# Fabstir/fabstir-vectordb

Measured on AMD Instinct MI355X. Metric: k-NN queries/sec at recall@10>=0.95, 1Mx384 f32, higher is better.
Workload: dtype f32

## Files before the change

### fabstir-vectordb_amd/csrc/fvdb_hip.cpp

```cpp
#include "fvdb_internal.h"

#include <unistd.h>

#include <algorithm>
#include <atomic>
#include <cmath>
#include <condition_variable>
#include <mutex>
#include <cstdio>
#include <cstdlib>
#include <cstring>
#include <map>
#include <new>
#include <string>
#include <vector>

#include "common.h"
#include "pool.h"
#include "kernels_misc.h"
#include "kernels_scan.h"
#include "kernels_wide.h"
#include "kernels_range.h"
#include "kernels_rank.h"
#include "kernels_curve.h"
#include "kernels_coarse.h"
#include "kernels_mfma.h"
#include "kernels_mfma_wg.h"
#include "kernels_util.h"
#include "kernels_maint.h"
#include "kernels_rows.h"
#include "kernels_mmr.h"
#include "kernels_group.h"

using namespace fvdb;


enum FbWord : uint32_t {
  FB_COARSE = 0,
  FB_SCAN = 1,
  FB_REASONS = 2,
  FB_OVERFLOW = 2,
  FB_REFINED = 6,
  FB_WORDS = 8,
};
constexpr size_t kFbBytes = FB_WORDS * 4;
constexpr size_t kFbAllBytes = 2 * kFbBytes;
constexpr uint32_t kFbReasonWords = 5;

enum StageEvent {
  EV_COARSE_BEGIN = 0,
  EV_COARSE_SCANNED,
  EV_COARSE_DONE,
  EV_SCAN_BEGIN,
  EV_SCAN_DONE,
  EV_FINE_DONE,
  EV_FILTER_BEGIN,
  EV_FILTER_DONE,
  EV_COUNT
};

enum ScalWord : uint32_t {
  SC_COARSE_ITEMS = 0,
  SC_COARSE_HEAD = 1,
  SC_FINE_ITEMS = 2,
  SC_FINE_HEAD = 3,
  SC_STATS = 4,
};
constexpr size_t kScalarsBytes = 64;

struct IvfScratch {
  std::mutex enq;
  bool pend_filter = false;
  bool pending_profile = false, pend_coarse = false, pend_fine = false, collecting = false;
  DBuf s_qnorm, s_A;
  DBuf s_qh, s_qn2, s_thr, s_tA, s_pa, s_surv, s_scnt, s_fail, s_mslots;
  DBuf s_sdist, s_probes2;
  DBuf s_q, s_cpart, s_probes, s_cnt, s_fill, s_eoff, s_ioff, s_entries;
  DBuf s_part, s_scalars, s_ceoff, s_cioff;
  DBuf s_wbase, s_arena;
  DBuf s_wgbase;
  DBuf s_gwords, s_group;
  DBuf s_rbase, s_rarena;
  DBuf s_qual;
  DBuf s_clive, s_cprobes, s_ckeys, s_cval;
  DBuf s_in, s_slots, s_ids, s_clusters, s_out_ids, s_out_dist, s_out_cnt, s_cdist;
  DBuf s_fslots, s_frows;
  DevEvent fetch_done;
  DevEvent sev[EV_COUNT];
  uint32_t* scalar(ScalWord w) const { return s_scalars.as<uint32_t>() + w; }
};

struct fvdb_ivf : IvfScratch {
  static constexpr uint32_t kSlots = 16;
  IvfScratch spare[kSlots - 1];
  static constexpr uint32_t kLeases = 8;
  IvfScratch lease_set[kLeases];
  fvdb_ctx* lease_ctx[kLeases] = {};
  uint32_t lease_busy = 0;
  std::mutex mu;
  std::condition_variable lease_cv;
  std::atomic<IvfScratch*> last_set{nullptr};
  std::atomic<fvdb_ctx*> last_ctx{nullptr};
  fvdb_ctx* ctx = nullptr;
  uint32_t d = 0, dpad = 0, d4 = 0, nlist = 0;
  bool trained = false;
  bool f16 = false;

  std::vector<float> h_centroids;
  DBuf d_centroids_rm;
  DBuf d_cent_pad;
  DBuf d_cnorm, d_cnmax;
  DBuf s_fallbacks;
  uint32_t* fb_word(FbWord w, bool masked = false) const { return s_fallbacks.as<uint32_t>() + (masked ? FB_WORDS : 0) + w; }
  int coarse_mode = 0;
  int scan_mode = 0;
  HBuf h_fb;
  uint64_t mfma_q = 0;
  uint64_t fb_seen = 0, q_seen = 0;
  uint32_t exact_batches_left = 0;
  uint32_t backoff_len = 0;
  uint64_t overflow_seen = 0, overflow_q = 0;
  uint32_t refine_batches_left = 0;
  DBuf d_mfma_stamps;
  int mfma_stamps_launch = 0;
  DBuf d_xmax;
  Pool cpool;
  DBuf c_off, c_blocks, c_glob;

  Pool pool;
// ... 8 lines not shown
  bool glob_set = false;

  DBuf m_seq, m_dest, m_ids;
  fvdb_ivf* m_src = nullptr;
  uint64_t m_rows = 0;
  bool m_assigned = false;
  bool m_store_job = false;
  fvdb_maintenance_info_t m_info{};

  fvdb_search_stats last_stats{};
  float stage_ms[8] = {0, 0, 0, 0, 0, 0, 0, 0};
  uint64_t stage_calls = 0;
};

namespace {
struct Env {
  fvdb_ctx* ctx;
  IvfScratch* S;
  const uint64_t* live = nullptr;
};
inline IvfScratch& slot_scratch(fvdb_ivf* ivf, uint32_t slot) { return slot == 0 ? *ivf : ivf->spare[slot - 1]; }
inline const uint64_t* live_words(const fvdb_ivf* ivf, const Env& E) { return E.live ? E.live : ivf->pool.valid(); }
inline PoolView list_pool(const fvdb_ivf* ivf, const Env& E) {
  PoolView v = ivf->pool.view();
  v.valid = live_words(ivf, E);
  return v;
}
}


namespace {

struct IvfKnobs {
  static int num(const char* name, int unset) { return getenv(name) ? atoi(getenv(name)) : unset; }
  static bool has(const char* name) { return getenv(name) != nullptr; }
  static int tiles(int m) { return m >= 4 ? 4 : (m >= 2 ? 2 : 1); }
  bool coarse_exact = has("FVDB_COARSE_EXACT");
  bool scan_exact = has("FVDB_SCAN_EXACT");
  uint32_t scan_wgs_per_cu = (uint32_t)num("FVDB_SCAN_WGS_PER_CU", 8);
  int segb = num("FVDB_SEGB", 0);
  bool no_shared_thr = has("FVDB_NO_SHARED_THR");
  int mfma_m = tiles(num("FVDB_MFMA_M", 2));
  int mfma_segb = num("FVDB_MFMA_SEGB", 0);
  uint32_t mfma_wgs_per_cu = (uint32_t)std::max(1, num("FVDB_MFMA_WGS_PER_CU", 2));
  bool mfma_groups_in_item = num("FVDB_MFMA_GROUPS_IN_ITEM", 0) != 0;
  bool mfma_wg = num("FVDB_MFMA_WG", 1) != 0;
  int mfma_wg_m = num("FVDB_MFMA_WG_M", 4) >= 4 ? 4 : 2;
  uint32_t mfma_wg_segb = (uint32_t)std::max(4, num("FVDB_MFMA_WG_SEGB", 16));
  uint32_t mfma_wg_per_cu = (uint32_t)std::max(1, num("FVDB_MFMA_WG_PER_CU", 2));
  int mfma_wg_tail_pct = num("FVDB_MFMA_WG_TAIL_PCT", 25);
  int mfma_wg_segb_tail = num("FVDB_MFMA_WG_SEGB_TAIL", 4);
  uint32_t mfma_cap_a = (uint32_t)std::max(1, num("FVDB_MFMA_CAP_A", 4));
  bool mfma_threshold_pass = has("FVDB_MFMA_THRESHOLD_PASS");
  uint32_t mfma_segb_a = (uint32_t)std::max(1, num("FVDB_MFMA_SEGB_A", 1));
  bool mfma_no_refine = has("FVDB_MFMA_NO_REFINE");
#ifdef FVDB_MFMA_STAMPS_BUILD
  int mfma_stamps = num("FVDB_MFMA_STAMPS", 0);
#endif
};
const IvfKnobs& ivf_knobs() {
  static const IvfKnobs knobs{};
  return knobs;
}

struct ScanLaunch {
  PoolView pool;
  const uint32_t* list_off;
  const uint32_t* list_blocks;
  uint32_t nlist;
  const uint32_t* entry_off;
  const uint32_t* item_off;
  const uint2* entries;
  const uint32_t* n_items;
  uint32_t* head;
  const float* queries;
  uint32_t dpad, segb, k, nprobe, maxsegs;
  uint2* part;
  uint32_t max_items = 0;
  bool f16 = false;
};

inline int kr_for(uint32_t k) { return k <= 64 ? 1 : (k <= 128 ? 2 : 4); }
inline uint32_t q_for(uint32_t k) { return k <= 64 ? 16u : (k <= 128 ? 8u : 4u); }

template <int Q, int KR, int ROLE, int ST>
void launch_scan_t(fvdb_ctx* ctx, const ScanLaunch& s) {
  uint32_t grid = (uint32_t)ctx->num_cus * ivf_knobs().scan_wgs_per_cu;
  if (s.max_items) grid = std::min(grid, std::max<uint32_t>(1u, (s.max_items + 3) / 4));
  hipLaunchKernelGGL((scan_topk_kernel<Q, KR, ROLE, ST>), dim3(grid), dim3(256), 0, ctx->stream, s.pool.data, s.pool.valid,
                     s.pool.d4, s.list_off, s.list_blocks, s.nlist, s.entry_off, s.item_off, (const u32x2*)s.entries,
                     s.n_items, s.head, s.queries, s.dpad, s.segb, s.k, s.nprobe, s.maxsegs, (u32x2*)s.part);
}

template <int ROLE, int ST>
void launch_scan_rs(fvdb_ctx* ctx, const ScanLaunch& s) {
  switch (kr_for(s.k)) {
    case 1: launch_scan_t<16, 1, ROLE, ST>(ctx, s); break;
    case 2: launch_scan_t<8, 2, ROLE, ST>(ctx, s); break;
    default: launch_scan_t<4, 4, ROLE, ST>(ctx, s); break;
  }
}
template <int ROLE>
void launch_scan_r(fvdb_ctx* ctx, const ScanLaunch& s) {
  if (s.f16) launch_scan_rs<ROLE, 1>(ctx, s); else launch_scan_rs<ROLE, 0>(ctx, s);
}
enum { ROLE_COARSE = 0, ROLE_LIST = 1, ROLE_ALL = 2 };
// ... 288 lines not shown
constexpr uint32_t kMfmaSlack = 6;
constexpr uint32_t kMfmaCmax = 4096;

bool mfma_shape_ok(const fvdb_ivf* ivf, uint32_t B, uint32_t k, uint32_t np) {
  return ivf->dpad % 16 == 0 && k + kMfmaSlack <= 32 && np <= 256 && B >= 32 && B <= 16384;
}
inline bool half_rows(const fvdb_ivf* ivf) { return ivf->f16 || ivf->pool.half() != nullptr; }
inline int x_rounded(const fvdb_ivf* ivf) { return ivf->f16 ? 0 : (ivf->pool.half() ? 1 : 2); }

struct MfmaPlan {
  bool wg;
  int M;
  uint32_t Q, ka, cmax;
  uint32_t segb, segbA;
  uint32_t lsplit, segb_tail;
  uint32_t fsegb, fmaxsegs;
  uint64_t fpart;
  uint32_t grid, wg_grid, wg_lds;
  bool half_rows;
  int x_rounded;
};

int mfma_plan(fvdb_ivf* ivf, fvdb_ctx* ctx, const IvfKnobs& kn, uint32_t B, uint32_t k, uint32_t np, MfmaPlan* out) {
  MfmaPlan P{};
  P.half_rows = half_rows(ivf);
  P.x_rounded = x_rounded(ivf);
  int wgM = kn.mfma_wg_m;
  if (mfma_wg_lds_bytes(ivf->dpad, 16u * wgM) > 64u * 1024u) wgM = 2;
  P.wg = kn.mfma_wg && kn.mfma_m == 2 && P.half_rows && ivf->dpad % 128 == 0 &&
         mfma_wg_lds_bytes(ivf->dpad, 16u * wgM) <= 64u * 1024u;
  P.M = P.wg ? wgM : kn.mfma_m;
  P.Q = 16u * P.M;
  P.ka = k + kMfmaSlack;
  P.cmax = kMfmaCmax;
  P.segbA = kn.mfma_segb_a;
  P.segb = P.wg ? kn.mfma_wg_segb : (kn.mfma_segb > 0 ? (uint32_t)kn.mfma_segb : pick_segb(ivf, B, np));
  P.lsplit = 0xFFFFFFFFu;
  P.segb_tail = P.segb;
  if (P.wg && kn.mfma_wg_tail_pct > 0 && kn.mfma_wg_segb_tail > 0 && (uint32_t)kn.mfma_wg_segb_tail < P.segb) {
    P.lsplit = (uint32_t)((uint64_t)ivf->nlist * (uint32_t)(100 - std::min(kn.mfma_wg_tail_pct, 100)) / 100);
    P.segb_tail = (uint32_t)kn.mfma_wg_segb_tail;
  }
  P.fsegb = pick_segb(ivf, B, np);
  P.fmaxsegs = std::max<uint32_t>(1, cdiv(ivf->max_list_blocks, P.fsegb));
  P.fpart = (uint64_t)B * np * P.fmaxsegs * k;
  if (P.fpart >= (1ull << 32)) FAIL(ctx, FVDB_E_UNSUPPORTED, "batch too large for one launch (sub-batch it)");
  P.grid = (uint32_t)ctx->num_cus * kn.mfma_wgs_per_cu;
  P.wg_grid = (uint32_t)ctx->num_cus * kn.mfma_wg_per_cu;
  P.wg_lds = mfma_wg_lds_bytes(ivf->dpad, P.Q);
  *out = P;
  return FVDB_OK;
}

int mfma_scratch(fvdb_ivf* ivf, const Env& E, const MfmaPlan& P, uint32_t B, uint32_t np) {
  fvdb_ctx* ctx = E.ctx;
  IvfScratch& S = *E.S;
  HIPCHK(ctx, S.s_qh.ensure((size_t)(B + 1) * ivf->dpad * 2));
  HIPCHK(ctx, S.s_qn2.ensure((size_t)B * 4));
  HIPCHK(ctx, S.s_thr.ensure((size_t)B * 4));
  HIPCHK(ctx, S.s_tA.ensure((size_t)B * 4));
  HIPCHK(ctx, S.s_pa.ensure((size_t)B * 4));
  HIPCHK(ctx, S.s_mslots.ensure((size_t)B * 64 * 4));
  HIPCHK(ctx, S.s_surv.ensure((size_t)B * P.cmax * 8));
  HIPCHK(ctx, S.s_sdist.ensure((size_t)B * P.cmax * 4));
  HIPCHK(ctx, S.s_scnt.ensure((size_t)(B + 2) * 4));
  HIPCHK(ctx, S.s_fail.ensure((size_t)B * 4));
  HIPCHK(ctx, S.s_part.ensure((size_t)P.fpart * 8));
  int rc = plan_scratch(ivf, E, B, np);
  if (rc) return rc;
  HIPCHK(ctx, S.s_scalars.ensure(kScalarsBytes));
  return FVDB_OK;
}

void launch_prep_queries(fvdb_ivf* ivf, const Env& E, const float* qpad, uint32_t B) {
  IvfScratch& S = *E.S;
  hipLaunchKernelGGL(prep_queries_kernel, dim3(cdiv(B + 1, 4)), dim3(256), 0, E.ctx->stream, qpad, B, ivf->dpad,
                     (_Float16*)S.s_qh.p, S.s_qn2.as<float>(), S.s_cnt.as<uint32_t>(), ivf->nlist,
                     S.s_scnt.as<uint32_t>(), S.s_mslots.as<uint32_t>());
}

ThresholdArgs threshold_args(fvdb_ivf* ivf, const Env& E, const float* qpad, const uint32_t* probes, uint32_t B,
                             uint32_t k, uint32_t np, float* thr_out) {
  const IvfScratch& S = *E.S;
  ThresholdArgs t{};
  t.rows = ivf->pool.half() ? ivf->pool.half() : ivf->pool.data();
  t.pool_valid = live_words(ivf, E);
  t.pool_norms = ivf->pool.norms();
  t.d4 = ivf->d4;
  t.lists = list_table(ivf);
  t.list_len = ivf->t_len.as<uint32_t>();
  t.probes = probes;
  t.qh = (const _Float16*)S.s_qh.p;
  t.queries = qpad;
  t.qn = S.s_qn2.as<float>();
  t.xmax_bits = ivf->d_xmax.as<uint32_t>();
  t.B = B;
  t.np = np;
  t.ka = k + kMfmaSlack;
  t.dpad = ivf->dpad;
  t.capA = ivf_knobs().mfma_cap_a;
  t.min_rows = 256u;
  t.rows_f16 = x_rounded(ivf);
  t.thr = thr_out;
  return t;
}
void launch_threshold_direct(fvdb_ivf* ivf, fvdb_ctx* ctx, const ThresholdArgs& t) {
  if (half_rows(ivf)) hipLaunchKernelGGL((threshold_direct_kernel<true>), dim3(cdiv(t.B, 4)), dim3(256), 0, ctx->stream, t);
  else hipLaunchKernelGGL((threshold_direct_kernel<false>), dim3(cdiv(t.B, 4)), dim3(256), 0, ctx->stream, t);
}

MfmaScanArgs mfma_scan_args(fvdb_ivf* ivf, const Env& E, const MfmaPlan& P, const Batch& b) {
  const IvfScratch& S = *E.S;
  MfmaScanArgs a{};
  a.pool_data = ivf->pool.half() ? ivf->pool.half() : ivf->pool.data();
  a.pool_valid = live_words(ivf, E);
  a.pool_norms = ivf->pool.norms();
  a.d4 = ivf->d4;
  a.list_off = ivf->t_off.as<uint32_t>();
  a.list_blocks = ivf->t_blocks.as<uint32_t>();
  a.nlist = ivf->nlist;
  a.entry_off = S.s_eoff.as<uint32_t>();
  a.item_off = S.s_ioff.as<uint32_t>();
  a.entries = (const u32x2*)S.s_entries.p;
  a.n_items = S.scalar(SC_FINE_ITEMS);
  a.head = S.scalar(SC_FINE_HEAD);
  a.qh = (const _Float16*)S.s_qh.p;
  a.zero_row = b.B;
  a.dpad = ivf->dpad;
  a.segb = P.segb;
  a.thr = b.given_thr ? b.given_thr : S.s_thr.as<float>();
  a.cmax = P.cmax;
  a.surv = (u32x2*)S.s_surv.p;
  a.sval = S.s_sdist.as<float>();
  a.scnt = S.s_scnt.as<uint32_t>();
  a.slots = S.s_mslots.as<uint32_t>();
  a.capA = ivf_knobs().mfma_cap_a;
  a.groups_in_item = ivf_knobs().mfma_groups_in_item ? 1u : 0u;
  a.lsplit = P.lsplit;
  a.segb_tail = P.segb_tail;
  return a;
}

using MfmaKernel = decltype(&scan_mfma_kernel<2, 1, 0>);
template <int M, int MODE>
MfmaKernel mfma_kernel_of(bool f16) {
  return f16 ? scan_mfma_kernel<M, 1, MODE> : scan_mfma_kernel<M, 0, MODE>;
}
template <int MODE>
void launch_mfma(fvdb_ctx* ctx, const MfmaScanArgs& a, const MfmaPlan& P) {
  const MfmaKernel kernel = P.M == 1   ? mfma_kernel_of<1, MODE>(P.half_rows)
                            : P.M == 2 ? mfma_kernel_of<2, MODE>(P.half_rows)
                                       : mfma_kernel_of<4, MODE>(P.half_rows);
  hipLaunchKernelGGL(kernel, dim3(P.grid), dim3(256), 0, ctx->stream, a);
}

void mfma_threshold(fvdb_ivf* ivf, const Env& E, const MfmaPlan& P, const Batch& b, const MfmaScanArgs& a) {
  fvdb_ctx* ctx = E.ctx;
  IvfScratch& S = *E.S;
  if (b.given_thr) return;
  if (!ivf_knobs().mfma_threshold_pass) {
    launch_threshold_direct(ivf, ctx, threshold_args(ivf, E, b.qpad, b.probes, b.B, b.k, b.np, S.s_thr.as<float>()));
    return;
  }
  hipLaunchKernelGGL(first_probe_kernel, dim3(cdiv(b.B, 256)), dim3(256), 0, ctx->stream, b.probes, b.B, b.np,
                     ivf->t_len.as<uint32_t>(), 256u, S.s_pa.as<uint32_t>());
  launch_plan(ivf, E, S.s_pa.as<uint32_t>(), b.B, 1, P.segbA, P.Q, nullptr, S.s_cnt.as<uint32_t>());
  MfmaScanArgs head = a;
  head.segb = P.segbA;
  launch_mfma<1>(ctx, head, P);
  hipLaunchKernelGGL(threshold_kernel, dim3(cdiv(b.B, 4)), dim3(256), 0, ctx->stream, S.s_mslots.as<uint32_t>(),
                     S.s_pa.as<uint32_t>(), S.s_qn2.as<float>(), ivf->d_xmax.as<uint32_t>(), b.B, P.ka, ivf->dpad,
                     P.x_rounded, S.s_thr.as<float>());
}

void launch_filter(fvdb_ctx* ctx, const MfmaScanArgs& a, const MfmaPlan& P) {
  if (P.wg) {
    const MfmaKernel kernel = P.M == 4 ? scan_mfma_wg_kernel<4> : scan_mfma_wg_kernel<2>;
    hipLaunchKernelGGL(kernel, dim3(P.wg_grid), dim3(256), P.wg_lds, ctx->stream, a);
  } else {
    launch_mfma<0>(ctx, a, P);
  }
}

#ifdef FVDB_MFMA_STAMPS_BUILD
constexpr uint32_t kStampsCap = 32768;
int mfma_stamps_begin(fvdb_ivf* ivf, fvdb_ctx* ctx, const MfmaPlan& P, MfmaScanArgs* a) {
  const int stamps_env = ivf_knobs().mfma_stamps;
  const bool stamp_now = P.wg && stamps_env && ++ivf->mfma_stamps_launch >= stamps_env && ivf->mfma_stamps_launch < stamps_env + 3;
  if (!stamp_now) return FVDB_OK;
  HIPCHK(ctx, ivf->d_mfma_stamps.ensure((size_t)kStampsCap * 64));
  HIPCHK(ctx, hipMemsetAsync(ivf->d_mfma_stamps.p, 0, (size_t)kStampsCap * 64, ctx->stream));
  a->stamps = ivf->d_mfma_stamps.as<unsigned long long>();
  a->stamps_cap = kStampsCap;
  return FVDB_OK;
}
int mfma_stamps_report(fvdb_ivf* ivf, fvdb_ctx* ctx, MfmaScanArgs* a) {
  if (!a->stamps) return FVDB_OK;
  HIPCHK(ctx, hipStreamSynchronize(ctx->stream));
  std::vector<unsigned long long> h((size_t)kStampsCap * 8);
  HIPCHK(ctx, hipMemcpy(h.data(), a->stamps, h.size() * 8, hipMemcpyDeviceToHost));
  unsigned long long t_min = ~0ull, t_max = 0;
  size_t n = 0;
  for (size_t i = 0; i < kStampsCap; ++i)
    if (h[i * 8 + 3]) {
      t_min = std::min(t_min, h[i * 8]);
      t_max = std::max(t_max, h[i * 8 + 3]);
      ++n;
    }
  double s_loc = 0, s_tile = 0, s_comp = 0, s_steps = 0, s_blocks = 0;
  size_t per_xcd[16] = {0};
  std::vector<double> per_step;
  for (size_t i = 0; i < kStampsCap; ++i) {
    const unsigned long long* r = &h[i * 8];
    if (!r[3]) continue;
// ... 128 lines not shown
}

FallbackArgs fallback_args(fvdb_ivf* ivf, const Env& E, const MfmaPlan& P, const Batch& b, const VerifyArgs& v) {
  const IvfScratch& S = *E.S;
  FallbackArgs fa{};
  fa.pool = list_pool(ivf, E);
  fa.lists = v.lists;
  fa.probes = b.probes;
  fa.queries = b.qpad;
  fa.fail_list = v.fail_list;
  fa.nfail = v.nfail;
  fa.head = S.s_scnt.as<uint32_t>() + b.B + 1;
  fa.k = b.k;
  fa.nprobe = b.np;
  fa.dpad = ivf->dpad;
  fa.segb = P.fsegb;
  fa.maxsegs = P.fmaxsegs;
  fa.part = (u32x2*)S.s_part.p;
  return fa;
}

void mfma_rescan(fvdb_ivf* ivf, const Env& E, const MfmaPlan& P, const Batch& b, const VerifyArgs& v) {
  fvdb_ctx* ctx = E.ctx;
  const FallbackArgs fa = fallback_args(ivf, E, P, b, v);
  if (ivf->f16) hipLaunchKernelGGL((fallback_scan_kernel<1>), dim3(P.grid), dim3(256), 0, ctx->stream, fa);
  else hipLaunchKernelGGL((fallback_scan_kernel<0>), dim3(P.grid), dim3(256), 0, ctx->stream, fa);
  MergeArgs fm = merge_args(fa.pool, fa.lists, v.glob_blocks, E.S->s_part, P.fmaxsegs, P.fsegb, b);
  fm.qlist = v.fail_list;
  fm.nq = v.nfail;
  launch_merge(ctx, fm);
}

int mfma_watch_counters(fvdb_ivf* ivf, fvdb_ctx* ctx, uint32_t B) {
  {
    std::lock_guard<std::mutex> lk(ivf->mu);
    const bool fresh = ivf->h_fb.p == nullptr;
    HIPCHK(ctx, ivf->h_fb.ensure(64));
    if (fresh) std::memset(ivf->h_fb.p, 0, 64);
    ivf->mfma_q += B;
  }
  HIPCHK(ctx, hipMemcpyAsync(ivf->h_fb.p, ivf->s_fallbacks.p, kFbBytes, hipMemcpyDeviceToHost, ctx->stream));
  return FVDB_OK;
}

int run_fine_mfma(fvdb_ivf* ivf, const Env& E, const Batch& b) {
  fvdb_ctx* ctx = E.ctx;
  const IvfKnobs& kn = ivf_knobs();
  MfmaPlan P;
  int rc = mfma_plan(ivf, ctx, kn, b.B, b.k, b.np, &P);
  if (rc) return rc;
  rc = mfma_scratch(ivf, E, P, b.B, b.np);
  if (rc) return rc;
  mark(ivf, E, EV_SCAN_BEGIN);
  launch_prep_queries(ivf, E, b.qpad, b.B);
  MfmaScanArgs a = mfma_scan_args(ivf, E, P, b);
  mfma_threshold(ivf, E, P, b, a);
  rc = mfma_filter(ivf, E, P, b, &a);
  if (rc) return rc;
  if (!b.given_thr && !kn.mfma_no_refine && (ivf->scan_mode != FVDB_SCAN_AUTO || auto_refines(ivf))) {
    rc = mfma_refine(ivf, E, P, b, a);
    if (rc) return rc;
  }
  mark(ivf, E, EV_SCAN_DONE);
  E.S->pend_filter = true;
  const VerifyArgs v = verify_args(ivf, E, P, b);
  launch_select(ivf, ctx, v);
  mfma_rescan(ivf, E, P, b, v);
  mark(ivf, E, EV_FINE_DONE);
  if (!E.live) {
    rc = mfma_watch_counters(ivf, ctx, b.B);
    if (rc) return rc;
  }
  HIPCHK(ctx, hipGetLastError());
  return FVDB_OK;
}

int run_fine(fvdb_ivf* ivf, const Env& E, const Batch& b, int role) {
  E.S->pend_filter = false;
  bool mfma = (ivf->scan_mode == FVDB_SCAN_AUTO || ivf->scan_mode == FVDB_SCAN_FILTER) && !ivf_knobs().scan_exact &&
              mfma_shape_ok(ivf, b.B, b.k, b.np) && role == ROLE_LIST && ivf->pool.norms() != nullptr;
  if (mfma && E.live && ivf->scan_mode == FVDB_SCAN_AUTO) mfma = false;
  if (mfma && ivf->scan_mode == FVDB_SCAN_AUTO && auto_backs_off(ivf)) mfma = false;
  if (mfma) return run_fine_mfma(ivf, E, b);
  return run_fine_exact(ivf, E, b, role);
}

struct StageSpan {
  StageEvent from, to;
};
constexpr StageSpan kStageSpan[6] = {
    {EV_COARSE_BEGIN, EV_COARSE_SCANNED}, {EV_COARSE_SCANNED, EV_COARSE_DONE},
    {EV_COARSE_DONE, EV_SCAN_BEGIN},
    {EV_SCAN_BEGIN, EV_SCAN_DONE},        {EV_SCAN_DONE, EV_FINE_DONE},
    {EV_FILTER_BEGIN, EV_FILTER_DONE}};

int finish_profile(fvdb_ivf* ivf, const Env& E, bool coarse, bool fine) {
  fvdb_ctx* ctx = E.ctx;
  IvfScratch& S = *E.S;
  if (!ivf->ctx->profiling) return FVDB_OK;
  if (ivf->ctx->profiling == 2 && !S.collecting) {
    S.pend_coarse = coarse;
    S.pend_fine = fine;
    S.pending_profile = true;
    return FVDB_OK;
  }
  HIPCHK(ctx, hipStreamSynchronize(ctx->stream));
  float ms = 0;
// ... 92 lines not shown
  } else if (b.glob_keys) {
    HIPCHK(ctx, S.s_wgbase.ensure((size_t)b.B * b.np * 4));
    hipLaunchKernelGGL(wide_gbase_kernel, dim3(cdiv(b.B, 256)), dim3(256), 0, ctx->stream, b.probes, ivf->t_glob.as<uint32_t>(),
                       b.B, b.np, S.s_wgbase.as<uint32_t>());
    w.gbase = S.s_wgbase.as<uint32_t>();
    if (b.np <= kWideMaxProbes)
      hipLaunchKernelGGL((wide_select_kernel<true, true>), dim3(b.B), dim3(kWideSelThreads), 0, ctx->stream, w);
    else
      hipLaunchKernelGGL((wide_select_kernel<false, true>), dim3(b.B), dim3(kWideSelThreads), 0, ctx->stream, w);
  } else if (b.np <= kWideMaxProbes)
    hipLaunchKernelGGL(wide_select_kernel<true>, dim3(b.B), dim3(kWideSelThreads), 0, ctx->stream, w);
  else
    hipLaunchKernelGGL(wide_select_kernel<false>, dim3(b.B), dim3(kWideSelThreads), 0, ctx->stream, w);
  mark(ivf, E, EV_FINE_DONE);
  HIPCHK(ctx, hipGetLastError());
  return FVDB_OK;
}

bool thr_share_ok(fvdb_ivf* ivf, uint32_t B, uint32_t k, uint32_t np) {
  const IvfKnobs& kn = ivf_knobs();
  if (kn.scan_exact || kn.no_shared_thr || ivf->scan_mode != FVDB_SCAN_AUTO) return false;
  if (!mfma_shape_ok(ivf, B, k, np)) return false;
  uint32_t gmax = 0;
  if (ivf->glob_set) {
    for (uint32_t b : ivf->glob_blocks_host) gmax = std::max(gmax, b);
  } else {
    gmax = ivf->max_list_blocks;
  }
  return queries_per_gib(gmax, segb_for(gmax, B, np), k, np) >= B;
}

int ivf_shared_thresholds(fvdb_ivf* ivf, const Env& E, const float* q_dev, const uint32_t* probes, uint32_t B, uint32_t k,
                          uint32_t np, float* u_out) {
  fvdb_ctx* ctx = E.ctx;
  IvfScratch& S = *E.S;
  HIPCHK(ctx, hipSetDevice(ctx->device));
  int rc = upload_table(ivf);
  if (rc) return rc;
  std::lock_guard<std::mutex> enq(S.enq);
  HIPCHK(ctx, S.s_qn2.ensure((size_t)B * 4));
  if (!ivf->pool.norms() || !ivf->d_xmax.p) {
    HIPCHK(ctx, hipMemsetAsync(S.s_qn2.p, 0, (size_t)B * 4, ctx->stream));
    hipLaunchKernelGGL(fill_f32_kernel, dim3(cdiv(B, 256)), dim3(256), 0, ctx->stream, u_out, (uint64_t)B, __builtin_huge_valf());
    HIPCHK(ctx, hipGetLastError());
    return FVDB_OK;
  }
  const float* qpad = nullptr;
  rc = padded_queries(ivf, E, q_dev, B, &qpad);
  if (rc) return rc;
  HIPCHK(ctx, S.s_qh.ensure((size_t)(B + 1) * ivf->dpad * 2));
  HIPCHK(ctx, S.s_cnt.ensure((size_t)ivf->nlist * 4));
  HIPCHK(ctx, S.s_scnt.ensure((size_t)(B + 2) * 4));
  HIPCHK(ctx, S.s_mslots.ensure((size_t)B * 64 * 4));
  launch_prep_queries(ivf, E, qpad, B);
  ThresholdArgs t = threshold_args(ivf, E, qpad, probes, B, k, np, u_out);
  t.glob_blocks = ivf->t_glob.as<uint32_t>();
  launch_threshold_direct(ivf, ctx, t);
  HIPCHK(ctx, hipGetLastError());
  return FVDB_OK;
}

int ivf_thr_combine(fvdb_ivf* ivf, const Env& E, const float* u_all, uint32_t W, uint32_t B, float* thr_out,
                    bool loopback_fill = false) {
  fvdb_ctx* ctx = E.ctx;
  IvfScratch& S = *E.S;
  if (!ivf->d_xmax.p) {
    HIPCHK(ctx, ivf->d_xmax.ensure(4));
    HIPCHK(ctx, hipMemsetAsync(ivf->d_xmax.p, 0, 4, ctx->stream));
  }
  hipLaunchKernelGGL(thr_combine_kernel, dim3(cdiv(B, 256)), dim3(256), 0, ctx->stream, u_all, W, B, S.s_qn2.as<float>(),
                     ivf->d_xmax.as<uint32_t>(), (float)ivf->dpad, x_rounded(ivf), thr_out);
#ifdef FVDB_DEV_TOOLS
  if (loopback_fill)
    hipLaunchKernelGGL(thr_loopback_fill_kernel, dim3(1), dim3(1024), 0, ctx->stream, thr_out, S.s_qn2.as<float>(), B);
#else
  (void)loopback_fill;
#endif
  HIPCHK(ctx, hipGetLastError());
  return FVDB_OK;
}

int check_finite(fvdb_ctx* ctx, const float* x, uint64_t n) {
  for (uint64_t i = 0; i < n; ++i)
    if (!std::isfinite(x[i])) FAIL(ctx, FVDB_E_NONFINITE, "non-finite input value");
  return FVDB_OK;
}

}

static std::mutex g_hwq_mu;
static int g_hwq_state = 0, g_hwq_value = 0;
static bool hip_runtime_already_up() {
  char path[64], tgt[256];
  for (int fd = 0; fd < 1024; ++fd) {
    snprintf(path, sizeof path, "/proc/self/fd/%d", fd);
    const ssize_t n = readlink(path, tgt, sizeof tgt - 1);
    if (n <= 0) continue;
    tgt[n] = 0;
    if (strstr(tgt, "/dev/kfd")) return true;
  }
  return false;
}

extern "C" {

const char* fvdb_version(void) { return "fvdb-hip 0.1 (gfx950)"; }

int fvdb_ctx_create(int device, fvdb_ctx** out) {
  if (!out) return FVDB_E_INVALID;
// ... 1797 lines not shown
```

### fabstir-vectordb_amd/csrc/kernels_mfma.h

```cpp
#pragma once
#include "score_rows.h"
#include "common.h"
#include "kernels_scan.h"

#pragma clang fp contract(off)

#ifndef FVDB_MFMA_WAVES
#define FVDB_MFMA_WAVES 2
#endif

namespace fvdb {

typedef _Float16 h8v __attribute__((ext_vector_type(8)));
typedef __fp16 fp16x2v __attribute__((ext_vector_type(2)));
typedef uint32_t u32x4v __attribute__((ext_vector_type(4)));
__device__ __forceinline__ uint32_t pk_rtz(float a, float b) {
  return __builtin_bit_cast(uint32_t, __builtin_amdgcn_cvt_pkrtz(a, b));
}
typedef float f32x16m __attribute__((ext_vector_type(16)));

constexpr float kHalfMax = 65504.0f;

__global__ void pool_row_norms_kernel(const float* __restrict__ src, uint32_t d, uint64_t n, int f16,
                                      const uint32_t* __restrict__ dst_slot, float* __restrict__ norms,
                                      uint32_t* __restrict__ xmax_bits) {
  const uint64_t i = (uint64_t)blockIdx.x * blockDim.x + threadIdx.x;
  if (i >= n) return;
  const float* r = src + i * d;
  float s = 0.0f;
  for (uint32_t j = 0; j < d; ++j) {
    const float v = f16 ? (float)(_Float16)r[j] : r[j];
    s = __builtin_fmaf(v, v, s);
  }
  norms[dst_slot[i]] = s;
  atomicMax(xmax_bits, __float_as_uint(s));
}

__global__ __launch_bounds__(256) void prep_queries_kernel(const float* __restrict__ q, uint32_t B, uint32_t dpad,
                                                           _Float16* __restrict__ qh, float* __restrict__ qn,
                                                           uint32_t* __restrict__ cnt, uint32_t nlist,
                                                           uint32_t* __restrict__ scnt, uint32_t* __restrict__ slots) {
  {
    const uint32_t gid = blockIdx.x * blockDim.x + threadIdx.x, gsz = gridDim.x * blockDim.x;
    for (uint32_t i = gid; i < nlist; i += gsz) cnt[i] = 0;
    for (uint32_t i = gid; i < B + 2; i += gsz) scnt[i] = 0;
    for (uint32_t i = gid; i < 64 * B; i += gsz) slots[i] = 0xFFFFFFFFu;
  }
  const int lane = threadIdx.x & 63;
  const uint32_t b = blockIdx.x * 4 + (threadIdx.x >> 6);
  if (b > B) return;
  if (b == B) {
    for (uint32_t j = lane; j < dpad; j += 64) qh[(size_t)b * dpad + j] = (_Float16)0.0f;
    return;
  }
  const float* r = q + (size_t)b * dpad;
  float s = 0.0f;
  for (uint32_t j = 2 * lane; j < dpad; j += 128) {
    const float a = r[j], c = r[j + 1];
    s = __builtin_fmaf(a, a, s);
    s = __builtin_fmaf(c, c, s);
    qh[(size_t)b * dpad + j] = (_Float16)a;
    qh[(size_t)b * dpad + j + 1] = (_Float16)c;
  }
#pragma unroll
  for (int o = 32; o > 0; o >>= 1) s += __shfl_xor(s, o);
  if (lane == 0) qn[b] = s;
}


__device__ __forceinline__ uint32_t fmap_u32(float v) {
  const uint32_t b = __float_as_uint(v);
  if (v != v) return 0u;
  return (b & 0x80000000u) ? ~b : (b | 0x80000000u);
}
__device__ __forceinline__ float funmap_u32(uint32_t u) {
  return __uint_as_float((u & 0x80000000u) ? (u & 0x7FFFFFFFu) : ~u);
}

__global__ void first_probe_kernel(const uint32_t* __restrict__ probes, uint32_t B, uint32_t np,
                                   const uint32_t* __restrict__ list_len, uint32_t min_rows,
                                   uint32_t* __restrict__ out) {
  const uint32_t b = blockIdx.x * blockDim.x + threadIdx.x;
  if (b >= B) return;
  uint32_t best = kInf32, best_len = 0;
  for (uint32_t r = 0; r < np; ++r) {
    const uint32_t L = probes[(size_t)b * np + r];
    if (L == kInf32) continue;
    const uint32_t len = list_len[L];
    if (len > best_len) {
      best = L;
      best_len = len;
    }
    if (len >= min_rows) break;
  }
  out[b] = best;
}

struct MfmaScanArgs {
  const void* pool_data;
  const uint64_t* pool_valid;
  const float* pool_norms;
  uint32_t d4;
  const uint32_t* list_off;
  const uint32_t* list_blocks;
  uint32_t nlist;
  const uint32_t* entry_off;
  const uint32_t* item_off;
  const u32x2* entries;
  const uint32_t* n_items;
  uint32_t* head;
  const _Float16* qh;
  uint32_t zero_row;
  uint32_t dpad, segb;
  const float* thr;
  uint32_t cmax;
  u32x2* surv;
  float* sval;
  uint32_t* scnt;
  uint32_t* slots;
// ... 337 lines not shown
}

__device__ __forceinline__ float mfma_error_bound(float xmax2, float qn2, float d, int x_rounded) {
  const float xm = sqrtf(xmax2) * 1.000001f, nq = sqrtf(qn2) * 1.000001f;
  if (!(xm < kHalfMax && nq < kHalfMax)) return __builtin_huge_valf();
  const float u10 = 9.765625e-4f, u11 = 4.8828125e-4f, u14 = 6.103515625e-5f, u24 = 5.9604645e-8f;
  const float ux = x_rounded == 0 ? 0.0f : (x_rounded == 1 ? u11 : u10);
  const float rnd = ux + u11 + ux * u11;
  const float e1 = 2.0f * rnd * xm * nq;
  const float e2 = 2.0f * (2.0f * d * u24) * xm * nq;
  const float e3 = 1.01f * (2.0f * d + 16.0f) * u24 * (xm + nq) * (xm + nq);
  const float e4 = 2.0f * u14 * sqrtf(d) * (xm + nq);
  return 1.05f * (e1 + e2 + e3 + e4) + 1e-6f * (xm + nq) * (xm + nq);
}

__global__ __launch_bounds__(256) void threshold_kernel(const uint32_t* __restrict__ slots, const uint32_t* __restrict__ first,
                                                        const float* __restrict__ qn,
                                                        const uint32_t* __restrict__ xmax_bits, uint32_t B, uint32_t ka,
                                                        uint32_t d, int rows_f16, float* __restrict__ thr_out) {
  const int lane = threadIdx.x & 63;
  const uint32_t q = rfl(blockIdx.x * 4 + (threadIdx.x >> 6));
  if (q >= B) return;
  const float inf = __builtin_huge_valf();
  float out = inf;
  if (first[q] != kInf32) {
    uint32_t hi = slots[(size_t)q * 64 + lane], lo = (uint32_t)lane;
    wave_sort64(hi, lo, lane);
    const uint32_t kth = rlane(hi, ka - 1);
    const float E = mfma_error_bound(__uint_as_float(*xmax_bits), qn[q], (float)d, rows_f16);
    if (kth != kInf32 && kth != 0u && E < inf) {
      const float a = funmap_u32(kth);
      out = a + 2.0f * E + 1e-6f * fabsf(a);
    }
  }
  if (lane == 0) thr_out[q] = out;
}

struct ThresholdArgs {
  const void* rows;
  const uint64_t* pool_valid;
  const float* pool_norms;
  uint32_t d4;
  ListTable lists;
  const uint32_t* list_len;
  const uint32_t* probes;
  const _Float16* qh;
  const float* queries;
  const float* qn;
  const uint32_t* xmax_bits;
  uint32_t B, np, ka, dpad, capA, min_rows;
  int rows_f16;
  float* thr;
  const uint32_t* glob_blocks;
};

template <bool HALF>
__global__ __launch_bounds__(256) void threshold_direct_kernel(const ThresholdArgs a) {
  const int lane = threadIdx.x & 63;
  const uint32_t q = rfl(blockIdx.x * 4 + (threadIdx.x >> 6));
  if (q >= a.B) return;
  const float inf = __builtin_huge_valf();
  uint32_t best_l = kInf32, best_len = 0;
  for (uint32_t r0 = 0; r0 < a.np && best_len < a.min_rows; r0 += 64) {
    const uint32_t r = r0 + lane;
    uint32_t L = kInf32, len = 0;
    if (r < a.np) {
      L = a.probes[(size_t)q * a.np + r];
      len = L != kInf32 ? (a.glob_blocks ? a.glob_blocks[L] * 64u : a.list_len[L]) : 0u;
    }
    const uint64_t big = __ballot(len >= a.min_rows);
    if (big) {
      const uint32_t l0 = (uint32_t)__builtin_ctzll(big);
      best_l = rlane(L, l0);
      best_len = rlane(len, l0);
      break;
    }
    uint32_t ml = len, mi = (uint32_t)lane;
#pragma unroll
    for (int o = 32; o > 0; o >>= 1) {
      const uint32_t ol = __shfl_xor(ml, o), oi = __shfl_xor(mi, o);
      if (ol > ml || (ol == ml && oi < mi)) {
        ml = ol;
        mi = oi;
      }
    }
    ml = rfl(ml);
    if (ml > best_len) {
      best_len = ml;
      best_l = rlane(L, rfl(mi));
    }
  }
  float out = inf;
  if (best_l != kInf32 && best_len > 0) {
    const uint32_t b_begin = cload(a.lists.off + best_l);
    const uint32_t nblk = min(cload(a.lists.off + best_l + 1) - b_begin, a.capA);
    float best = inf;
    bool bad = false;
    const uint32_t n8 = a.dpad >> 3;
    for (uint32_t b = 0; b < nblk; ++b) {
      const uint32_t blk = cload(a.lists.blocks + b_begin + b);
      float dot = 0.0f;
      if (HALF) {
        const h8v* xp = (const h8v*)a.rows + (size_t)blk * n8 * 64 + lane;
        const _Float16* qrow = a.qh + (size_t)q * a.dpad;
#pragma unroll 4
        for (uint32_t c = 0; c < n8; ++c) {
          const h8v x = xp[(size_t)c * 64];
          const h8v qv = cload((const h8v*)(qrow + 8 * c));
          typedef _Float16 h2v __attribute__((ext_vector_type(2)));
#pragma unroll
          for (int t = 0; t < 4; ++t)
            dot = __builtin_amdgcn_fdot2(h2v{x[2 * t], x[2 * t + 1]}, h2v{qv[2 * t], qv[2 * t + 1]}, dot, false);
        }
      } else {
        const float4* xp = (const float4*)a.rows + (size_t)blk * a.d4 * 64 + lane;
        const float* qrow = a.queries + (size_t)q * a.dpad;
        for (uint32_t c = 0; c < a.d4; ++c) {
          const float4 x = xp[(size_t)c * 64];
          const f32x4 qv = cload((const f32x4*)(qrow + 4 * c));
          dot = __builtin_fmaf(x.x, qv[0], dot);
          dot = __builtin_fmaf(x.y, qv[1], dot);
          dot = __builtin_fmaf(x.z, qv[2], dot);
          dot = __builtin_fmaf(x.w, qv[3], dot);
        }
      }
      const bool live = (cload(a.pool_valid + blk) >> lane) & 1ull;
      const float v = __builtin_fmaf(-2.0f, dot, a.pool_norms[(size_t)blk * 64 + lane]);
      if (live) {
        if (v != v) bad = true;
        else if (v < best) best = v;
      }
    }
    if (!__ballot(bad)) {
      uint32_t hi = best < inf ? fmap_u32(best) : kInf32, lo = (uint32_t)lane;
      wave_sort64(hi, lo, lane);
      const uint32_t kth = rlane(hi, a.ka - 1);
      const float E = mfma_error_bound(__uint_as_float(*a.xmax_bits), a.qn[q], (float)a.dpad, a.rows_f16);
      if (kth != kInf32 && kth != 0u && E < inf) {
        const float av = funmap_u32(kth);
        out = av + (a.glob_blocks ? 1.0f : 2.0f) * E + 1e-6f * fabsf(av);
      }
    }
  }
  if (lane == 0) a.thr[q] = out;
}

__global__ void thr_combine_kernel(const float* __restrict__ u_all, uint32_t W, uint32_t n, const float* __restrict__ qn,
                                   const uint32_t* __restrict__ xmax_bits, float d, int rows_f16, float* __restrict__ thr) {
  const uint32_t i = blockIdx.x * blockDim.x + threadIdx.x;
  if (i >= n) return;
  float m = __builtin_huge_valf();
  for (uint32_t w = 0; w < W; ++w) m = fminf(m, u_all[(size_t)w * n + i]);
  thr[i] = m + mfma_error_bound(__uint_as_float(*xmax_bits), qn[i], d, rows_f16);
}
#ifdef FVDB_DEV_TOOLS
__global__ __launch_bounds__(1024) void thr_loopback_fill_kernel(float* __restrict__ thr, const float* __restrict__ qn, uint32_t n) {
  __shared__ float s_sum[1024];
  __shared__ uint32_t s_cnt[1024];
  float sum = 0.0f;
  uint32_t cnt = 0;
  for (uint32_t i = threadIdx.x; i < n; i += 1024) {
    const float t = thr[i];
    if (t < __builtin_huge_valf()) {
      sum += t + qn[i];
      cnt += 1;
    }
  }
  s_sum[threadIdx.x] = sum;
  s_cnt[threadIdx.x] = cnt;
  __syncthreads();
  for (uint32_t o = 512; o > 0; o >>= 1) {
    if (threadIdx.x < o) {
      s_sum[threadIdx.x] += s_sum[threadIdx.x + o];
      s_cnt[threadIdx.x] += s_cnt[threadIdx.x + o];
    }
    __syncthreads();
  }
  if (s_cnt[0] == 0) return;
  const float typ = s_sum[0] / (float)s_cnt[0];
  for (uint32_t i = threadIdx.x; i < n; i += 1024)
    if (!(thr[i] < __builtin_huge_valf())) thr[i] = typ - qn[i];
}
#endif

__global__ __launch_bounds__(256) void refine_threshold_kernel(const float* __restrict__ sval, uint32_t* __restrict__ scnt,
                                                               const uint32_t* __restrict__ probes, const float* __restrict__ qn,
                                                               const uint32_t* __restrict__ xmax_bits, uint32_t B, uint32_t np,
                                                               uint32_t ka, uint32_t cmax, uint32_t d, int rows_f16,
                                                               float* __restrict__ thr, uint32_t* __restrict__ probes2,
                                                               uint32_t* __restrict__ n_refined) {
  const int lane = threadIdx.x & 63;
  const uint32_t q = rfl(blockIdx.x * 4 + (threadIdx.x >> 6));
  if (q >= B) return;
  const float inf = __builtin_huge_valf();
  bool again = false;
  if (scnt[q] > cmax) {
    WaveTopK<1> ta;
// ... 266 lines not shown
```

Baseline: 1.908 million.

## Group queries sharing a threshold list so one wave scores several queries

Moves the per-query pick of the threshold list into prep_queries, then sorts queries by picked list in a single-block bitonic sort and forms items of up to G queries that share a list. A new grouped threshold kernel loads each list block once and computes dot products for all G queries, so row data is reused instead of being reloaded for every query. It adds a serial one-workgroup sort kernel and an extra launch, and limits grouping to B up to 16384 and a bounded nlist.

```diff
diff --git a/fabstir-vectordb_amd/csrc/fvdb_hip.cpp b/fabstir-vectordb_amd/csrc/fvdb_hip.cpp
--- a/fabstir-vectordb_amd/csrc/fvdb_hip.cpp
+++ b/fabstir-vectordb_amd/csrc/fvdb_hip.cpp
@@ -65,6 +65,7 @@
   SC_FINE_ITEMS = 2,
   SC_FINE_HEAD = 3,
   SC_STATS = 4,
+  SC_THR_ITEMS = 10,
 };
 constexpr size_t kScalarsBytes = 64;
 
@@ -75,6 +76,7 @@
   DBuf s_qnorm, s_A;
   DBuf s_qh, s_qn2, s_thr, s_tA, s_pa, s_surv, s_scnt, s_fail, s_mslots;
   DBuf s_sdist, s_probes2;
+  DBuf s_tpick, s_tkeys, s_titems;
   DBuf s_q, s_cpart, s_probes, s_cnt, s_fill, s_eoff, s_ioff, s_entries;
   DBuf s_part, s_scalars, s_ceoff, s_cioff;
   DBuf s_wbase, s_arena;
@@ -189,6 +191,8 @@
   int mfma_wg_segb_tail = num("FVDB_MFMA_WG_SEGB_TAIL", 4);
   uint32_t mfma_cap_a = (uint32_t)std::max(1, num("FVDB_MFMA_CAP_A", 4));
   bool mfma_threshold_pass = has("FVDB_MFMA_THRESHOLD_PASS");
+  static int group(int g) { return g == 0 || g == 4 || g == 8 ? g : 8; }
+  int mfma_threshold_group = group(num("FVDB_MFMA_THRESHOLD_GROUP", 8));
   uint32_t mfma_segb_a = (uint32_t)std::max(1, num("FVDB_MFMA_SEGB_A", 1));
   bool mfma_no_refine = has("FVDB_MFMA_NO_REFINE");
 #ifdef FVDB_MFMA_STAMPS_BUILD
@@ -583,6 +587,21 @@
   return FVDB_OK;
 }
 
+int threshold_group(const fvdb_ivf* ivf, uint32_t B) {
+  const IvfKnobs& kn = ivf_knobs();
+  if (kn.mfma_threshold_pass || B > kThrGroupMaxB || ivf->nlist > kThrGroupMaxLists) return 0;
+  return kn.mfma_threshold_group;
+}
+int threshold_group_scratch(fvdb_ivf* ivf, const Env& E, uint32_t B) {
+  fvdb_ctx* ctx = E.ctx;
+  IvfScratch& S = *E.S;
+  if (!threshold_group(ivf, B)) return FVDB_OK;
+  HIPCHK(ctx, S.s_tpick.ensure((size_t)B * 4));
+  HIPCHK(ctx, S.s_tkeys.ensure((size_t)B * 4));
+  HIPCHK(ctx, S.s_titems.ensure((size_t)B * 4));
+  return FVDB_OK;
+}
+
 int mfma_scratch(fvdb_ivf* ivf, const Env& E, const MfmaPlan& P, uint32_t B, uint32_t np) {
   fvdb_ctx* ctx = E.ctx;
   IvfScratch& S = *E.S;
@@ -599,19 +618,21 @@
   HIPCHK(ctx, S.s_part.ensure((size_t)P.fpart * 8));
   int rc = plan_scratch(ivf, E, B, np);
   if (rc) return rc;
+  rc = threshold_group_scratch(ivf, E, B);
+  if (rc) return rc;
   HIPCHK(ctx, S.s_scalars.ensure(kScalarsBytes));
   return FVDB_OK;
 }
 
-void launch_prep_queries(fvdb_ivf* ivf, const Env& E, const float* qpad, uint32_t B) {
+void launch_prep_queries(fvdb_ivf* ivf, const Env& E, const float* qpad, uint32_t B, const ThresholdPick& pick) {
   IvfScratch& S = *E.S;
   hipLaunchKernelGGL(prep_queries_kernel, dim3(cdiv(B + 1, 4)), dim3(256), 0, E.ctx->stream, qpad, B, ivf->dpad,
                      (_Float16*)S.s_qh.p, S.s_qn2.as<float>(), S.s_cnt.as<uint32_t>(), ivf->nlist,
-                     S.s_scnt.as<uint32_t>(), S.s_mslots.as<uint32_t>());
+                     S.s_scnt.as<uint32_t>(), S.s_mslots.as<uint32_t>(), pick);
 }
 
 ThresholdArgs threshold_args(fvdb_ivf* ivf, const Env& E, const float* qpad, const uint32_t* probes, uint32_t B,
-                             uint32_t k, uint32_t np, float* thr_out) {
+                             uint32_t k, uint32_t np, float* thr_out, const uint32_t* glob_blocks = nullptr) {
   const IvfScratch& S = *E.S;
   ThresholdArgs t{};
   t.rows = ivf->pool.half() ? ivf->pool.half() : ivf->pool.data();
@@ -633,11 +654,27 @@
   t.min_rows = 256u;
   t.rows_f16 = x_rounded(ivf);
   t.thr = thr_out;
+  t.glob_blocks = glob_blocks;
+  if (threshold_group(ivf, B)) {
+    t.pick = S.s_tpick.as<uint32_t>();
+    t.skeys = S.s_tkeys.as<uint32_t>();
+    t.items = S.s_titems.as<uint32_t>();
+    t.n_items = S.scalar(SC_THR_ITEMS);
+  }
   return t;
 }
+using ThresholdKernel = decltype(&threshold_direct_kernel<true>);
 void launch_threshold_direct(fvdb_ivf* ivf, fvdb_ctx* ctx, const ThresholdArgs& t) {
-  if (half_rows(ivf)) hipLaunchKernelGGL((threshold_direct_kernel<true>), dim3(cdiv(t.B, 4)), dim3(256), 0, ctx->stream, t);
-  else hipLaunchKernelGGL((threshold_direct_kernel<false>), dim3(cdiv(t.B, 4)), dim3(256), 0, ctx->stream, t);
+  const bool half = half_rows(ivf);
+  ThresholdKernel kernel = half ? threshold_direct_kernel<true> : threshold_direct_kernel<false>;
+  if (t.pick) {
+    const int G = threshold_group(ivf, t.B);
+    hipLaunchKernelGGL(threshold_groups_kernel, dim3(1), dim3(1024), 0, ctx->stream, t.pick, t.B, (uint32_t)G, t.skeys,
+                       t.items, t.n_items, t.thr);
+    if (G == 4) kernel = half ? threshold_grouped_kernel<true, 4> : threshold_grouped_kernel<false, 4>;
+    else kernel = half ? threshold_grouped_kernel<true, 8> : threshold_grouped_kernel<false, 8>;
+  }
+  hipLaunchKernelGGL(kernel, dim3(cdiv(t.B, 4)), dim3(256), 0, ctx->stream, t);
 }
 
 MfmaScanArgs mfma_scan_args(fvdb_ivf* ivf, const Env& E, const MfmaPlan& P, const Batch& b) {
@@ -685,12 +722,15 @@
   hipLaunchKernelGGL(kernel, dim3(P.grid), dim3(256), 0, ctx->stream, a);
 }
 
+ThresholdArgs mfma_threshold_args(fvdb_ivf* ivf, const Env& E, const Batch& b) {
+  return threshold_args(ivf, E, b.qpad, b.probes, b.B, b.k, b.np, E.S->s_thr.as<float>());
+}
 void mfma_threshold(fvdb_ivf* ivf, const Env& E, const MfmaPlan& P, const Batch& b, const MfmaScanArgs& a) {
   fvdb_ctx* ctx = E.ctx;
   IvfScratch& S = *E.S;
   if (b.given_thr) return;
   if (!ivf_knobs().mfma_threshold_pass) {
-    launch_threshold_direct(ivf, ctx, threshold_args(ivf, E, b.qpad, b.probes, b.B, b.k, b.np, S.s_thr.as<float>()));
+    launch_threshold_direct(ivf, ctx, mfma_threshold_args(ivf, E, b));
     return;
   }
   hipLaunchKernelGGL(first_probe_kernel, dim3(cdiv(b.B, 256)), dim3(256), 0, ctx->stream, b.probes, b.B, b.np,
@@ -925,7 +965,7 @@
   rc = mfma_scratch(ivf, E, P, b.B, b.np);
   if (rc) return rc;
   mark(ivf, E, EV_SCAN_BEGIN);
-  launch_prep_queries(ivf, E, b.qpad, b.B);
+  launch_prep_queries(ivf, E, b.qpad, b.B, b.given_thr ? ThresholdPick{} : threshold_pick_of(mfma_threshold_args(ivf, E, b)));
   MfmaScanArgs a = mfma_scan_args(ivf, E, P, b);
   mfma_threshold(ivf, E, P, b, a);
   rc = mfma_filter(ivf, E, P, b, &a);
@@ -1124,9 +1164,11 @@
   HIPCHK(ctx, S.s_cnt.ensure((size_t)ivf->nlist * 4));
   HIPCHK(ctx, S.s_scnt.ensure((size_t)(B + 2) * 4));
   HIPCHK(ctx, S.s_mslots.ensure((size_t)B * 64 * 4));
-  launch_prep_queries(ivf, E, qpad, B);
-  ThresholdArgs t = threshold_args(ivf, E, qpad, probes, B, k, np, u_out);
-  t.glob_blocks = ivf->t_glob.as<uint32_t>();
+  rc = threshold_group_scratch(ivf, E, B);
+  if (rc) return rc;
+  HIPCHK(ctx, S.s_scalars.ensure(kScalarsBytes));
+  const ThresholdArgs t = threshold_args(ivf, E, qpad, probes, B, k, np, u_out, ivf->t_glob.as<uint32_t>());
+  launch_prep_queries(ivf, E, qpad, B, threshold_pick_of(t));
   launch_threshold_direct(ivf, ctx, t);
   HIPCHK(ctx, hipGetLastError());
   return FVDB_OK;
diff --git a/fabstir-vectordb_amd/csrc/kernels_mfma.h b/fabstir-vectordb_amd/csrc/kernels_mfma.h
--- a/fabstir-vectordb_amd/csrc/kernels_mfma.h
+++ b/fabstir-vectordb_amd/csrc/kernels_mfma.h
@@ -36,15 +36,60 @@
   atomicMax(xmax_bits, __float_as_uint(s));
 }
 
+struct ThresholdPick {
+  const uint32_t* probes;
+  const uint32_t* list_len;
+  const uint32_t* glob_blocks;
+  uint32_t np, min_rows;
+  uint32_t* pick;
+  uint32_t* n_items;
+};
+
+__device__ __forceinline__ uint32_t threshold_pick_list(const ThresholdPick& p, uint32_t q, int lane) {
+  uint32_t best_l = kInf32, best_len = 0;
+  for (uint32_t r0 = 0; r0 < p.np && best_len < p.min_rows; r0 += 64) {
+    const uint32_t r = r0 + lane;
+    uint32_t L = kInf32, len = 0;
+    if (r < p.np) {
+      L = p.probes[(size_t)q * p.np + r];
+      len = L != kInf32 ? (p.glob_blocks ? p.glob_blocks[L] * 64u : p.list_len[L]) : 0u;
+    }
+    const uint64_t big = __ballot(len >= p.min_rows);
+    if (big) {
+      const uint32_t l0 = (uint32_t)__builtin_ctzll(big);
+      best_l = rlane(L, l0);
+      best_len = rlane(len, l0);
+      break;
+    }
+    uint32_t ml = len, mi = (uint32_t)lane;
+#pragma unroll
+    for (int o = 32; o > 0; o >>= 1) {
+      const uint32_t ol = __shfl_xor(ml, o), oi = __shfl_xor(mi, o);
+      if (ol > ml || (ol == ml && oi < mi)) {
+        ml = ol;
+        mi = oi;
+      }
+    }
+    ml = rfl(ml);
+    if (ml > best_len) {
+      best_len = ml;
+      best_l = rlane(L, rfl(mi));
+    }
+  }
+  return best_len > 0 ? best_l : kInf32;
+}
+
 __global__ __launch_bounds__(256) void prep_queries_kernel(const float* __restrict__ q, uint32_t B, uint32_t dpad,
                                                            _Float16* __restrict__ qh, float* __restrict__ qn,
                                                            uint32_t* __restrict__ cnt, uint32_t nlist,
-                                                           uint32_t* __restrict__ scnt, uint32_t* __restrict__ slots) {
+                                                           uint32_t* __restrict__ scnt, uint32_t* __restrict__ slots,
+                                                           const ThresholdPick tp) {
   {
     const uint32_t gid = blockIdx.x * blockDim.x + threadIdx.x, gsz = gridDim.x * blockDim.x;
     for (uint32_t i = gid; i < nlist; i += gsz) cnt[i] = 0;
     for (uint32_t i = gid; i < B + 2; i += gsz) scnt[i] = 0;
     for (uint32_t i = gid; i < 64 * B; i += gsz) slots[i] = 0xFFFFFFFFu;
+    if (gid == 0 && tp.pick) *tp.n_items = 0;
   }
   const int lane = threadIdx.x & 63;
   const uint32_t b = blockIdx.x * 4 + (threadIdx.x >> 6);
@@ -65,6 +110,10 @@
 #pragma unroll
   for (int o = 32; o > 0; o >>= 1) s += __shfl_xor(s, o);
   if (lane == 0) qn[b] = s;
+  if (tp.pick) {
+    const uint32_t L = threshold_pick_list(tp, b, lane);
+    if (lane == 0) tp.pick[b] = L;
+  }
 }
 
 
@@ -508,7 +557,15 @@
   int rows_f16;
   float* thr;
   const uint32_t* glob_blocks;
+  uint32_t* pick;
+  uint32_t* skeys;
+  uint32_t* items;
+  uint32_t* n_items;
 };
+
+__device__ __host__ __forceinline__ ThresholdPick threshold_pick_of(const ThresholdArgs& a) {
+  return ThresholdPick{a.probes, a.list_len, a.glob_blocks, a.np, a.min_rows, a.pick, a.n_items};
+}
 
 template <bool HALF>
 __global__ __launch_bounds__(256) void threshold_direct_kernel(const ThresholdArgs a) {
@@ -516,38 +573,9 @@
   const uint32_t q = rfl(blockIdx.x * 4 + (threadIdx.x >> 6));
   if (q >= a.B) return;
   const float inf = __builtin_huge_valf();
-  uint32_t best_l = kInf32, best_len = 0;
-  for (uint32_t r0 = 0; r0 < a.np && best_len < a.min_rows; r0 += 64) {
-    const uint32_t r = r0 + lane;
-    uint32_t L = kInf32, len = 0;
-    if (r < a.np) {
-      L = a.probes[(size_t)q * a.np + r];
-      len = L != kInf32 ? (a.glob_blocks ? a.glob_blocks[L] * 64u : a.list_len[L]) : 0u;
-    }
-    const uint64_t big = __ballot(len >= a.min_rows);
-    if (big) {
-      const uint32_t l0 = (uint32_t)__builtin_ctzll(big);
-      best_l = rlane(L, l0);
-      best_len = rlane(len, l0);
-      break;
-    }
-    uint32_t ml = len, mi = (uint32_t)lane;
-#pragma unroll
-    for (int o = 32; o > 0; o >>= 1) {
-      const uint32_t ol = __shfl_xor(ml, o), oi = __shfl_xor(mi, o);
-      if (ol > ml || (ol == ml && oi < mi)) {
-        ml = ol;
-        mi = oi;
-      }
-    }
-    ml = rfl(ml);
-    if (ml > best_len) {
-      best_len = ml;
-      best_l = rlane(L, rfl(mi));
-    }
-  }
+  const uint32_t best_l = threshold_pick_list(threshold_pick_of(a), q, lane);
   float out = inf;
-  if (best_l != kInf32 && best_len > 0) {
+  if (best_l != kInf32) {
     const uint32_t b_begin = cload(a.lists.off + best_l);
     const uint32_t nblk = min(cload(a.lists.off + best_l + 1) - b_begin, a.capA);
     float best = inf;
@@ -599,6 +627,180 @@
     }
   }
   if (lane == 0) a.thr[q] = out;
+}
+
+constexpr uint32_t kThrKeyQBits = 14;
+constexpr uint32_t kThrGroupMaxB = 1u << kThrKeyQBits;
+constexpr uint32_t kThrGroupMaxLists = (1u << (32 - kThrKeyQBits)) - 1;
+
+__global__ __launch_bounds__(1024) void threshold_groups_kernel(const uint32_t* __restrict__ pick, uint32_t B, uint32_t G,
+                                                                uint32_t* __restrict__ skeys, uint32_t* __restrict__ items,
+                                                                uint32_t* __restrict__ n_items, float* __restrict__ thr) {
+  __shared__ uint32_t key[kThrGroupMaxB];
+  const uint32_t tid = threadIdx.x;
+  uint32_t n = 64;
+  while (n < B) n <<= 1;
+  for (uint32_t i = tid; i < n; i += 1024) {
+    const uint32_t L = i < B ? pick[i] : kInf32;
+    key[i] = L != kInf32 ? (L << kThrKeyQBits | i) : kInf32;
+    if (i < B && L == kInf32) thr[i] = __builtin_huge_valf();
+  }
+  __syncthreads();
+  for (uint32_t k2 = 2; k2 <= n; k2 <<= 1) {
+    for (uint32_t j = k2 >> 1; j > 0; j >>= 1) {
+      for (uint32_t t = tid; t < (n >> 1); t += 1024) {
+        const uint32_t i = ((t & ~(j - 1)) << 1) | (t & (j - 1));
+        const uint32_t x = key[i], y = key[i + j];
+        if ((x > y) == ((i & k2) == 0)) {
+          key[i] = y;
+          key[i + j] = x;
+        }
+      }
+      __syncthreads();
+    }
+  }
+  const int lane = tid & 63;
+  for (uint32_t i0 = 0; i0 < n; i0 += 1024) {
+    const uint32_t i = i0 + tid;
+    const uint32_t kv = i < n ? key[i] : kInf32;
+    bool opens = false;
+    if (kv != kInf32) {
+      const uint32_t first_key = kv >> kThrKeyQBits << kThrKeyQBits;
+      uint32_t lo = 0, hi = i;
+      while (lo < hi) {
+        const uint32_t mid = (lo + hi) >> 1;
+        if (key[mid] < first_key) lo = mid + 1; else hi = mid;
+      }
+      opens = (i - lo) % G == 0;
+    }
+    if (i < B) skeys[i] = kv;
+    const uint64_t m = __ballot(opens);
+    if (m) {
+      uint32_t base = 0;
+      if (lane == 0) base = atomicAdd(n_items, (uint32_t)__builtin_popcountll(m));
+      base = rfl(base);
+      if (opens) items[base + (uint32_t)__builtin_popcountll(m & ((1ull << lane) - 1))] = i;
+    }
+  }
+}
+
+template <bool HALF>
+struct ThrChunk;
+template <>
+struct ThrChunk<true> {
+  typedef h8v X;
+  typedef _Float16 Q;
+  static constexpr uint32_t kDims = 8;
+  static __device__ __forceinline__ float dot(const X x, const Q* __restrict__ q, float dot) {
+    const h8v qv = cload((const h8v*)q);
+    typedef _Float16 h2v __attribute__((ext_vector_type(2)));
+#pragma unroll
+    for (int t = 0; t < 4; ++t)
+      dot = __builtin_amdgcn_fdot2(h2v{x[2 * t], x[2 * t + 1]}, h2v{qv[2 * t], qv[2 * t + 1]}, dot, false);
+    return dot;
+  }
+};
+template <>
+struct ThrChunk<false> {
+  typedef float4 X;
+  typedef float Q;
+  static constexpr uint32_t kDims = 4;
+  static __device__ __forceinline__ float dot(const X x, const Q* __restrict__ q, float dot) {
+    const f32x4 qv = cload((const f32x4*)q);
+    dot = __builtin_fmaf(x.x, qv[0], dot);
+    dot = __builtin_fmaf(x.y, qv[1], dot);
+    dot = __builtin_fmaf(x.z, qv[2], dot);
+    dot = __builtin_fmaf(x.w, qv[3], dot);
+    return dot;
+  }
+};
+
+constexpr int kThrLoads = 8;
+
+template <bool HALF, int G>
+__global__ __launch_bounds__(256) void threshold_grouped_kernel(const ThresholdArgs a) {
+  typedef ThrChunk<HALF> C;
+  const int lane = threadIdx.x & 63;
+  const uint32_t item = rfl(blockIdx.x * 4 + (threadIdx.x >> 6));
+  if (item >= cload(a.n_items)) return;
+  const float inf = __builtin_huge_valf();
+  const uint32_t start = cload(a.items + item);
+  const uint32_t key0 = cload(a.skeys + start);
+  const uint32_t list = key0 >> kThrKeyQBits;
+  uint32_t nq = 0;
+  const typename C::Q* qrow[G];
+  uint32_t qi[G];
+#pragma unroll
+  for (int g = 0; g < G; ++g) {
+    const uint32_t kv = start + g < a.B ? cload(a.skeys + start + g) : kInf32;
+    const bool mine = (kv >> kThrKeyQBits) == list && kv != kInf32;
+    qi[g] = (mine ? kv : key0) & (kThrGroupMaxB - 1);
+    qrow[g] = (HALF ? (const typename C::Q*)a.qh : (const typename C::Q*)a.queries) + (size_t)qi[g] * a.dpad;
+    nq += mine ? 1u : 0u;
+  }
+  const uint32_t b_begin = cload(a.lists.off + list);
+  const uint32_t nblk = min(cload(a.lists.off + list + 1) - b_begin, a.capA);
+  const uint32_t nch = HALF ? a.dpad >> 3 : a.d4;
+  float best[G];
+  bool bad[G];
+#pragma unroll
+  for (int g = 0; g < G; ++g) {
+    best[g] = inf;
+    bad[g] = false;
+  }
+  for (uint32_t b = 0; b < nblk; ++b) {
+    const uint32_t blk = cload(a.lists.blocks + b_begin + b);
+    const typename C::X* xp = (const typename C::X*)a.rows + (size_t)blk * nch * 64 + lane;
+    float dot[G];
+#pragma unroll
+    for (int g = 0; g < G; ++g) dot[g] = 0.0f;
+    uint32_t c = 0;
+    for (; c + kThrLoads <= nch; c += kThrLoads) {
+      typename C::X x[kThrLoads];
+#pragma unroll
+      for (int u = 0; u < kThrLoads; ++u) x[u] = xp[(size_t)(c + u) * 64];
+#pragma unroll
+      for (int g = 0; g < G; ++g) {
+        if ((uint32_t)g < nq) {
+#pragma unroll
+          for (int u = 0; u < kThrLoads; ++u) dot[g] = C::dot(x[u], qrow[g] + C::kDims * (c + u), dot[g]);
+        }
+      }
+    }
+    for (; c < nch; ++c) {
+      const typename C::X x = xp[(size_t)c * 64];
+#pragma unroll
+      for (int g = 0; g < G; ++g)
+        if ((uint32_t)g < nq) dot[g] = C::dot(x, qrow[g] + C::kDims * c, dot[g]);
+    }
+    const bool live = (cload(a.pool_valid + blk) >> lane) & 1ull;
+    const float norm = a.pool_norms[(size_t)blk * 64 + lane];
+#pragma unroll
+    for (int g = 0; g < G; ++g) {
+      const float v = __builtin_fmaf(-2.0f, dot[g], norm);
+      if (live && (uint32_t)g < nq) {
+        if (v != v) bad[g] = true;
+        else if (v < best[g]) best[g] = v;
+      }
+    }
+  }
+  const float xmax2 = __uint_as_float(*a.xmax_bits);
+#pragma unroll
+  for (int g = 0; g < G; ++g) {
+    if ((uint32_t)g >= nq) break;
+    float out = inf;
+    if (!__ballot(bad[g])) {
+      uint32_t hi = best[g] < inf ? fmap_u32(best[g]) : kInf32, lo = (uint32_t)lane;
+      wave_sort64(hi, lo, lane);
+      const uint32_t kth = rlane(hi, a.ka - 1);
+      const float E = mfma_error_bound(xmax2, a.qn[qi[g]], (float)a.dpad, a.rows_f16);
+      if (kth != kInf32 && kth != 0u && E < inf) {
+        const float av = funmap_u32(kth);
+        out = av + (a.glob_blocks ? 1.0f : 2.0f) * E + 1e-6f * fabsf(av);
+      }
+    }
+    if (lane == 0) a.thr[qi[g]] = out;
+  }
 }
 
 __global__ void thr_combine_kernel(const float* __restrict__ u_all, uint32_t W, uint32_t n, const float* __restrict__ qn,
```

Result: slower. 1.823 million (-4.5%).
